# jojolebarjos/board-game-simulator-python

Hardware: AMD Instinct MI355X
Metric: env-steps/sec, Connect4(6,7,4) random rollout, batch=2^20 per GPU (higher is better)
Workload: dtype u64

## Files before the change

board-game-simulator-python_amd/csrc/bgs_host.hip:

```cpp
#include <immintrin.h>
#include <limits.h>
#include <linux/futex.h>
#include <pthread.h>
#include <sched.h>
#include <sys/syscall.h>
#include <time.h>
#include <unistd.h>

#include <atomic>
#include <chrono>
#include <condition_variable>
#include <cstdlib>
#include <cstdio>
#include <algorithm>
#include <cstring>
#include <mutex>
#include <new>
#include <thread>
#include <vector>

#include "bgs_capi_util.h"
#include "bgs_common.h"
#include "bgs_internal.h"

struct bgs_event {
    int device;
    hipEvent_t ev;
};

namespace {

using bgs::fail;

struct ExpandTable {
    uint64_t pairs[256];
    ExpandTable() {
        for (int byte = 0; byte < 256; ++byte) {
            uint64_t four = 0;
            for (int j = 0; j < 4; ++j) four |= (uint64_t)bgs::reward_pair((uint32_t)(byte >> (2 * j)) & 3u) << (16 * j);
            pairs[byte] = four;
        }
    }
};
const ExpandTable g_expand;

template <bool STREAM>
__attribute__((target("avx2"))) int64_t expand_avx2(const uint8_t* src, int64_t code_bytes, int8_t* dst) {
    const __m256i spread = _mm256_setr_epi8(0, 0, 0, 0, 1, 1, 1, 1, 2, 2, 2, 2, 3, 3, 3, 3,
                                            4, 4, 4, 4, 5, 5, 5, 5, 6, 6, 6, 6, 7, 7, 7, 7);
    const __m256i field = _mm256_set1_epi32((int)0xC0300C03u);
    const __m256i one = _mm256_set1_epi32(0x40100401);
    const __m256i two = _mm256_set1_epi32((int)0x80200802u);
    int64_t i = 0;
    for (; i + 8 <= code_bytes; i += 8) {
        long long eight;
        memcpy(&eight, src + i, 8);
        const __m256i rep = _mm256_shuffle_epi8(_mm256_set1_epi64x(eight), spread);
        const __m256i f = _mm256_and_si256(rep, field);
        const __m256i is1 = _mm256_cmpeq_epi8(f, one), is2 = _mm256_cmpeq_epi8(f, two);
        const __m256i r0 = _mm256_sub_epi8(is2, is1), r1 = _mm256_sub_epi8(is1, is2);
        const __m256i lo = _mm256_unpacklo_epi8(r0, r1), hi = _mm256_unpackhi_epi8(r0, r1);
        const __m256i first = _mm256_permute2x128_si256(lo, hi, 0x20), second = _mm256_permute2x128_si256(lo, hi, 0x31);
        if (STREAM) {
            _mm256_stream_si256(reinterpret_cast<__m256i*>(dst + 8 * i), first);
            _mm256_stream_si256(reinterpret_cast<__m256i*>(dst + 8 * i + 32), second);
        } else {
            _mm256_storeu_si256(reinterpret_cast<__m256i*>(dst + 8 * i), first);
            _mm256_storeu_si256(reinterpret_cast<__m256i*>(dst + 8 * i + 32), second);
        }
    }
    if (STREAM) _mm_sfence();
    return i;
}

const bool g_have_avx2 = __builtin_cpu_supports("avx2");
const bool g_stream_stores = bgs::experiment("no_stream_stores") == nullptr;
// ... 122 lines not shown
    while (seen < value && !a->compare_exchange_weak(seen, value, std::memory_order_release, std::memory_order_relaxed)) {
    }
    if (seen < value) futex(word, FUTEX_WAKE, INT_MAX, nullptr);
}

bool device_node_cpus(int device, cpu_set_t* out) {
    CPU_ZERO(out);
    char bus[64] = {0};
    if (hipDeviceGetPCIBusId(bus, (int)sizeof bus, device) != hipSuccess) return false;
    for (char* c = bus; *c; ++c) *c = (char)tolower(*c);
    char path[256];
    snprintf(path, sizeof path, "/sys/bus/pci/devices/%s/numa_node", bus);
    FILE* f = fopen(path, "r");
    if (!f) return false;
    int node = -1;
    const int got = fscanf(f, "%d", &node);
    fclose(f);
    if (got != 1 || node < 0) return false;
    snprintf(path, sizeof path, "/sys/devices/system/node/node%d/cpulist", node);
    f = fopen(path, "r");
    if (!f) return false;
    char list[4096] = {0};
    const bool have = fgets(list, sizeof list, f) != nullptr;
    fclose(f);
    if (!have) return false;
    cpu_set_t allowed;
    if (sched_getaffinity(0, sizeof allowed, &allowed) != 0) return false;
    int any = 0;
    char* save = nullptr;
    for (char* tok = strtok_r(list, ",\n", &save); tok; tok = strtok_r(nullptr, ",\n", &save)) {
        int lo = 0, hi = 0;
        const int k = sscanf(tok, "%d-%d", &lo, &hi);
        if (k < 1) continue;
        if (k == 1) hi = lo;
        for (int c = lo; c <= hi && c < CPU_SETSIZE; ++c)
            if (CPU_ISSET(c, &allowed)) {
                CPU_SET(c, out);
                ++any;
            }
    }
    return any > 0;
}

}

namespace {
inline bool sink_trace_on() {
    static const bool on = bgs::experiment("sink_trace") != nullptr;
    return on;
}
inline double mono_us() {
    return std::chrono::duration<double, std::micro>(std::chrono::steady_clock::now().time_since_epoch()).count();
}
}

static bool codes_hold_a_zero(const uint8_t* codes, int64_t first, int64_t count) {
    const uint8_t* p = codes + first / 4;
    const int64_t whole = count / 4;
    int64_t i = 0;
    uint64_t seen = 0;
    for (; i + 8 <= whole; i += 8) {
        uint64_t x;
        memcpy(&x, p + i, 8);
        seen |= ~(x | (x >> 1)) & 0x5555555555555555ull;
    }
    for (; i < whole; ++i) seen |= (uint64_t)(~(p[i] | (p[i] >> 1)) & 0x55u);
    for (int64_t k = 0; k < count - whole * 4; ++k) seen |= ((p[whole] >> (2 * k)) & 3u) == 0u ? 1u : 0u;
    return seen != 0;
}

struct bgs_reward_sink {
    int device = 0;
    int64_t max_games = 0;
    int slots = 0;
    int ring = 0;
    int threads = 0;
    std::vector<uint8_t*> pinned;
    std::vector<uint8_t*> mapped;
    std::vector<hipEvent_t> landed;
    bool grids = false;
    CellFormat cells;
    size_t slot_bytes = 0;
    struct Job {
        int64_t n_games = 0;
        int8_t* host_reward = nullptr;
        int event_slot = 0;
        bool all_end = false;
    };
    std::vector<Job> jobs;
    std::mutex mu;
    std::condition_variable cv_submit;
    std::condition_variable cv_landed;
    std::condition_variable cv_done;
    int64_t claimed = 0;
    int64_t submitted = 0;
    volatile int64_t* progress = nullptr;
    int64_t landed_upto = 0;
    int64_t completed = 0;
    std::vector<int> parts_done;
    std::vector<char> slot_ok;
    bool stop = false;
    std::vector<int64_t> failed_tickets;
    bool poll = false;
    std::vector<std::thread> workers;
    std::atomic<int64_t> a_submitted{0}, a_landed{0}, a_completed{0};
    std::atomic<bool> a_stop{false};
    std::atomic<int> urgent{0};
    int spin_us = 0;
    int wait_spin_us = 200;

    bool spin_for(const std::atomic<int64_t>& counter, int64_t ticket) const {
        if (counter.load(std::memory_order_acquire) > ticket) return true;
        if (spin_us <= 0) return false;
        const auto until = std::chrono::steady_clock::now() + std::chrono::microseconds(spin_us);
        for (;;) {
            for (int i = 0; i < 64; ++i) {
                if (counter.load(std::memory_order_acquire) > ticket || a_stop.load(std::memory_order_relaxed)) return true;
                _mm_pause();
            }
            if (std::chrono::steady_clock::now() >= until) return false;
        }
// ... 7 lines not shown
            bool ok = true;
            if (t == 0) {
                spin_for(a_submitted, ticket);
                {
                    std::unique_lock<std::mutex> lock(mu);
                    cv_submit.wait(lock, [&] { return stop || submitted > ticket; });
                    if (submitted <= ticket) return;
                    job = jobs[slot];
                }
                if (job.n_games == 0) {
                    ok = false;
                } else if (poll || urgent.load(std::memory_order_relaxed) > 0) {
                    hipError_t e;
                    while ((e = hipEventQuery(landed[job.event_slot])) == hipErrorNotReady) _mm_pause();
                    ok = e == hipSuccess;
                } else {
                    ok = hipEventSynchronize(landed[job.event_slot]) == hipSuccess;
                }
                if (sink_trace_on()) fprintf(stderr, "sink-trace ticket %lld landed %.1f\n", (long long)ticket, mono_us());
                {
                    std::lock_guard<std::mutex> lock(mu);
                    if (!ok && job.n_games != 0) failed_tickets.push_back(ticket);
                    slot_ok[slot] = ok;
                    landed_upto = ticket + 1;
                    a_landed.store(ticket + 1, std::memory_order_release);
                }
                cv_landed.notify_all();
            } else {
                if (urgent.load(std::memory_order_relaxed) > 0) {
                    const auto until = std::chrono::steady_clock::now() + std::chrono::microseconds(2000);
                    while (a_landed.load(std::memory_order_acquire) <= ticket && !a_stop.load(std::memory_order_relaxed) &&
                           urgent.load(std::memory_order_relaxed) > 0 && std::chrono::steady_clock::now() < until)
                        for (int i = 0; i < 16; ++i) _mm_pause();
                } else {
                    spin_for(a_landed, ticket);
                }
                std::unique_lock<std::mutex> lock(mu);
                cv_landed.wait(lock, [&] { return stop || landed_upto > ticket; });
                if (landed_upto <= ticket) return;
                job = jobs[slot];
                ok = slot_ok[slot];
            }
            const int expanders = threads > 1 ? threads - 1 : 1;
            const int share = threads > 1 ? t - 1 : 0;
            if (threads > 1 && t == 0) continue;
            const double trace_t0 = sink_trace_on() ? mono_us() : 0.0;
            if (ok && grids) {
                const int64_t blocks = (job.n_games + 63) / 64;
                const int64_t g0 = blocks * share / expanders * 64;
                const int64_t g1 = share + 1 == expanders ? job.n_games : blocks * (share + 1) / expanders * 64;
                static const bool skip = bgs::experiment("grid_no_expand") != nullptr;
                if (g1 > g0 && !skip) expand_cells(pinned[slot], job.n_games, cells, g0, g1 - g0, job.host_reward);
            } else if (ok) {
                const int64_t bytes = (job.n_games + 3) / 4;
                const int64_t b0 = bytes * share / expanders, b1 = bytes * (share + 1) / expanders;
                const int64_t first = b0 * 4;
                int64_t count = b1 * 4 - first;
                if (first + count > job.n_games) count = job.n_games - first;
                if (count > 0) expand_range(pinned[slot], first, count, job.host_reward);
                if (count > 0 && job.all_end && codes_hold_a_zero(pinned[slot], first, count)) {
                    std::lock_guard<std::mutex> lock(mu);
                    if (std::find(failed_tickets.begin(), failed_tickets.end(), ticket) == failed_tickets.end()) failed_tickets.push_back(ticket);
                }
            }
            if (sink_trace_on()) fprintf(stderr, "sink-trace ticket %lld worker %d expand %.1f .. %.1f\n", (long long)ticket, t, trace_t0, mono_us());
            {
                std::lock_guard<std::mutex> lock(mu);
                if (++parts_done[slot] == expanders) {
                    parts_done[slot] = 0;
                    ++completed;
                    a_completed.store(completed, std::memory_order_release);
                    cv_done.notify_all();
                    if (progress) progress_store_max(progress, completed);
                }
            }
        }
    }
};

namespace {

int64_t claim(bgs_reward_sink* s, bool ahead = false) {
    const int bound = ahead ? s->ring : s->slots;
    s->spin_for(s->a_completed, s->a_submitted.load(std::memory_order_relaxed) - bound);
    std::unique_lock<std::mutex> lock(s->mu);
    s->cv_done.wait(lock, [&] { return s->claimed - s->completed < bound; });
    return s->claimed++;
}

void publish(bgs_reward_sink* s, int64_t ticket, int64_t n_games, int8_t* host_reward, bool ok = true, int64_t event_ticket = -1,
             bool all_end = false) {
    {
        std::unique_lock<std::mutex> lock(s->mu);
        s->cv_done.wait(lock, [&] { return s->submitted == ticket; });
        s->jobs[ticket % s->ring].n_games = ok ? n_games : 0;
        s->jobs[ticket % s->ring].all_end = all_end;
        s->jobs[ticket % s->ring].host_reward = host_reward;
        s->jobs[ticket % s->ring].event_slot = (int)((event_ticket >= 0 ? event_ticket : ticket) % s->ring);
        if (!ok) s->failed_tickets.push_back(ticket);
        s->submitted = ticket + 1;
        s->a_submitted.store(ticket + 1, std::memory_order_release);
    }
    s->cv_submit.notify_one();
    s->cv_done.notify_all();
}

}

namespace bgs {
int64_t sink_claim(bgs_reward_sink* s) { return claim(s); }
uint8_t* sink_slot_device(bgs_reward_sink* s, int64_t ticket) { return s->mapped[ticket % s->ring]; }
uint8_t* sink_slot_host(bgs_reward_sink* s, int64_t ticket) { return s->pinned[ticket % s->ring]; }
hipEvent_t sink_slot_event(bgs_reward_sink* s, int64_t ticket) { return s->landed[ticket % s->ring]; }
void sink_publish(bgs_reward_sink* s, int64_t ticket, int64_t n_games, int8_t* host_reward, bool ok, int64_t event_ticket, bool all_end) {
    publish(s, ticket, n_games, host_reward, ok, event_ticket, all_end);
}
bool sink_takes_group(const bgs_reward_sink* s, int count) { return s != nullptr && !s->grids && count <= s->ring; }
int sink_ring(const bgs_reward_sink* s) { return s->ring; }
int sink_rollout_group(bgs_reward_sink* s, bgs_batch* const* bs, const uint64_t* seeds, const bool* writes, int count,
                       hipStream_t stream, int8_t* const* host_rewards, int64_t* tickets) {
    NEED(count >= 1 && count <= kConnectGroupMax && count <= s->ring && !s->grids, "bad step group");
    for (int i = 0; i < count; ++i)
        NEED(bs[i]->device == s->device && bs[i]->n <= s->max_games, "the batch does not fit the sink");
    uint32_t* codes[kConnectGroupMax];
    for (int i = 0; i < count; ++i) {
        tickets[i] = claim(s, true);
        codes[i] = reinterpret_cast<uint32_t*>(s->mapped[tickets[i] % s->ring]);
    }
    connect_rollout_steps(bs, seeds, codes, writes, count, stream);
    hipError_t err = hipGetLastError();
    if (err == hipSuccess) err = hipEventRecord(s->landed[tickets[count - 1] % s->ring], stream);
    for (int i = 0; i < count; ++i) publish(s, tickets[i], bs[i]->n, host_rewards[i], err == hipSuccess, tickets[count - 1]);
    if (err != hipSuccess) return fail(BGS_ERR_RUNTIME, "grouped rollout could not be enqueued: %s", hipGetErrorString(err));
    return BGS_OK;
}
int sink_wait(bgs_reward_sink* s, int64_t ticket, bool urgent) {
    NEED(s != nullptr, "sink is NULL");
    NEED(ticket >= 0 && ticket < s->a_submitted.load(std::memory_order_acquire), "unknown ticket %lld", (long long)ticket);
    if (s->a_completed.load(std::memory_order_acquire) <= ticket) {
        if (urgent) {
            s->urgent.fetch_add(1, std::memory_order_relaxed);
            const auto until = std::chrono::steady_clock::now() + std::chrono::microseconds(s->wait_spin_us);
            while (s->a_completed.load(std::memory_order_acquire) <= ticket && std::chrono::steady_clock::now() < until)
                for (int i = 0; i < 32; ++i) _mm_pause();
        } else {
            s->spin_for(s->a_completed, ticket);
        }
        {
            std::unique_lock<std::mutex> lock(s->mu);
            s->cv_done.wait(lock, [&] { return s->completed > ticket; });
        }
        if (urgent) s->urgent.fetch_sub(1, std::memory_order_relaxed);
    }
    int64_t bad = -1;
    {
        std::lock_guard<std::mutex> lock(s->mu);
        auto& f = s->failed_tickets;
        for (size_t i = 0; i < f.size();) {
            if (f[i] <= ticket) {
                if (bad < 0 || f[i] < bad) bad = f[i];
                f.erase(f.begin() + (long)i);
            } else {
                ++i;
            }
        }
    }
    if (bad >= 0)
        return fail(BGS_ERR_RUNTIME, "reward hand-over %lld failed (its enqueue, its arrival event, or -- a gathered step whose games all "
                    "had to end -- a rank delivered games that are still running: its step failed there); later deliveries are unaffected",
                    (long long)bad);
    return BGS_OK;
}
}

extern "C" {

int bgs_host_alloc(size_t bytes, void** host_ptr) {
    NEED(host_ptr != nullptr && bytes > 0, "bad argument");
    *host_ptr = nullptr;
    HIP_TRY(hipHostMalloc(host_ptr, bytes, hipHostMallocDefault));
    return BGS_OK;
}

int bgs_host_free(void* host_ptr) {
// ... 407 lines not shown
```

board-game-simulator-python_amd/csrc/bgs_internal.h:

```cpp
#pragma once

#include <hip/hip_runtime.h>
#include <stdint.h>
#include <stddef.h>

struct bgs_reward_sink;
struct bgs_gather;

enum { BGS_GAME_CONNECT = 1, BGS_GAME_BOUNCE = 2 };

#include "connect_unit.h"
#include "bounce_unit.h"

struct bgs_batch {
    int game;
    int generic;
    int gen_h, gen_w, gen_k;
    uint32_t gen_init_status;
    int device;
    int64_t n;
    hipStream_t stream;
    uint64_t first_game;
    ConnectGeom cg;
    BounceGeom bg;
    int planes;
    int num_cus;
    int rollout_wps;
    int bounce_group;
    int bounce_group_auto;
    int bounce_pieces;
    int bounce_flat_wps;
    int bounce_eval_wps;
    int bounce_flat_waves;
    int bounce_pool;
    int bounce_pieces_park;
    int bounce_park;
    int bounce_flat_chunk;
    int launches_in_flight;
    int bounce_memo_cold, bounce_memo_bypass;
    int bounce_epoch_limit;
    int bounce_wave_pass;
    int bounce_plan_auto;
    int bounce_passes;
    uint32_t bounce_pass_cap[BGS_BOUNCE_MAX_PASSES];
    int bounce_pass_group[BGS_BOUNCE_MAX_PASSES];
    int bounce_wave_grid;
    int transition_wave;
    int bounce_static_geom;
    int rollout_generic;
    int rollout_chunk;
    int rollout_opening;
    int rollout_no_lds;
    int rng_per_ply;
    void* arena;
    size_t arena_bytes;
    bool owns_arena;
    uint64_t* d_planes;
    uint8_t* d_status;
    uint16_t* d_plies;
    int8_t* d_reward;
    unsigned long long* d_steps;
    uint8_t* d_staging;
    size_t staging_bytes;
    uint64_t* d_gen_masks;
    int8_t* d_gen_cfg;
    uint32_t* d_worklist;
    uint32_t* d_work_count;
    uint32_t* d_pool;
    const uint32_t* book_links;
    const void* book_table;
    int book_depth;
    uint32_t book_n0;
    void* book_owner;
    void* pinned[2];
    hipEvent_t pinned_done[2];
    hipEvent_t order_event;
};

namespace bgs {

#ifdef BGS_TEST_HOOKS
const char* experiment(const char* name);
#else
inline const char* experiment(const char*) { return nullptr; }
#endif

void connect_reset(const bgs_batch* b);
void connect_step_random(const bgs_batch* b, uint64_t seed, uint32_t count);
void connect_step_actions(const bgs_batch* b, const int32_t* d_actions, int32_t* d_status_out);
bool connect_step_observe(const bgs_batch* b, const int32_t* d_actions, int32_t* d_status_out, uint8_t* d_legal, uint8_t* d_ended,
                          int8_t* d_reward_out, bool auto_reset);
void connect_reset_ended(const bgs_batch* b);
void bounce_reset_ended(const bgs_batch* b);
void status_to_ended(const bgs_batch* b, uint8_t* d_ended);
void connect_transition(const bgs_batch* b, const int32_t* d_actions, int32_t* d_status_out, int8_t* d_grid, int8_t* d_player,
                        int8_t* d_winner, int32_t* d_plies, uint8_t* d_legal, int8_t* d_reward_out, uint32_t* d_done = nullptr,
                        uint32_t ticket = 0);
bool connect_rollout(const bgs_batch* b, uint64_t seed, int32_t max_plies, uint32_t flags, uint32_t* codes_out);
bool connect_steps_ok(const bgs_batch* b, int32_t max_plies, uint32_t flags, bool codes);
void connect_rollout_steps(const bgs_batch* const* bs, const uint64_t* seeds, uint32_t* const* codes, const bool* writes, int count,
                           hipStream_t stream);
void connect_unpack_grid(const bgs_batch* b, int8_t* d_grid);
void connect_cell_planes(const bgs_batch* b, uint64_t* d_dst);
void connect_meta(const bgs_batch* b, int8_t* d_player, uint8_t* d_ended, int8_t* d_winner, int32_t* d_plies);
void connect_legal(const bgs_batch* b, uint8_t* d_legal, int32_t* d_count);
void connect_pack(const bgs_batch* b, const int8_t* d_grid, const int8_t* d_player, const int8_t* d_winner,
                  int32_t* d_status_out);

void connect_evaluate(const bgs_batch* b, uint64_t seed, int32_t playouts, int32_t max_plies, int32_t* d_counts, int policy);
int32_t connect_halving_min_budget(int width);
void connect_evaluate_halving(const bgs_batch* b, uint64_t seed, int32_t budget, int32_t max_plies, int policy, int32_t* d_counts,
                              int32_t* d_given, int32_t* d_best);
uint64_t connect_search_root_bytes(int width, int32_t iterations);
void connect_search(const bgs_batch* b, uint64_t seed, int32_t iterations, int32_t leaf_playouts, int32_t explore, int32_t max_plies,
                    int policy, int32_t* d_counts, int32_t* d_visits, int32_t* d_best, int32_t* d_nodes, void* d_workspace);
void connect_search_proving(const bgs_batch* b, uint64_t seed, int32_t iterations, int32_t leaf_playouts, int32_t explore,
                            int32_t max_plies, int policy, int32_t* d_counts, int32_t* d_visits, int32_t* d_best, int32_t* d_nodes,
                            int8_t* d_proved, int32_t* d_done, void* d_workspace);
uint64_t connect_forest_tree_bytes(int width, int32_t capacity);
void connect_forest_search(const bgs_batch* b, uint64_t seed, int32_t iterations, int32_t leaf_playouts, int32_t explore,
                           int32_t max_plies, int policy, int32_t capacity, int restart, int32_t* d_counts, int32_t* d_visits,
                           int32_t* d_best, int32_t* d_nodes, int32_t* d_carried, void* d_forest);
void connect_forest_advance(const bgs_batch* b, const int32_t* d_columns, int32_t capacity, int32_t* d_kept, void* d_forest);
uint64_t connect_guided_tree_bytes(int height, int width, int32_t capacity);
void connect_guided_step(const bgs_batch* b, int32_t capacity, int32_t cpuct, uint32_t flags, const float* d_priors,
                         const float* d_values, int8_t* d_leaf_grid, int8_t* d_leaf_player, int32_t* d_leaf_kind, int32_t* d_visits,
                         int32_t* d_scores, int32_t* d_best, int32_t* d_nodes, void* d_trees);
void connect_solve(const bgs_batch* b, int32_t depth, int64_t max_nodes, int8_t* d_codes, int16_t* d_plies,
                   unsigned long long* d_nodes);
void bounce_evaluate(const bgs_batch* b, uint64_t seed, int32_t playouts, int32_t max_plies, int32_t* d_counts, uint64_t* d_ends,
                     uint64_t* d_totals, int policy);
void bounce_evaluate_halving(const bgs_batch* b, uint64_t seed, int32_t budget, int32_t max_plies, int policy, int32_t* d_counts,
                             int32_t* d_given, int32_t* d_best);
uint64_t bounce_search_root_bytes(int32_t iterations, int32_t edges);
void bounce_search(const bgs_batch* b, uint64_t seed, int32_t iterations, int32_t leaf_playouts, int32_t explore, int32_t max_plies,
                   int policy, int32_t edges, int32_t* d_counts, int32_t* d_visits, int32_t* d_best, int32_t* d_nodes, int32_t* d_used,
                   void* d_workspace);
void bounce_search_proving(const bgs_batch* b, uint64_t seed, int32_t iterations, int32_t leaf_playouts, int32_t explore,
                           int32_t max_plies, int policy, int32_t edges, int32_t* d_counts, int32_t* d_visits, int32_t* d_best,
                           int32_t* d_nodes, int32_t* d_used, int8_t* d_proved, int32_t* d_done, void* d_workspace);
uint64_t bounce_forest_tree_bytes(int32_t capacity, int32_t edges);
void bounce_forest_search(const bgs_batch* b, uint64_t seed, int32_t iterations, int32_t leaf_playouts, int32_t explore,
                          int32_t max_plies, int policy, int32_t capacity, int32_t edges, int restart, int32_t* d_counts,
                          int32_t* d_visits, int32_t* d_best, int32_t* d_nodes, int32_t* d_used, int32_t* d_carried, void* d_forest);
void bounce_forest_advance(const bgs_batch* b, const int32_t* d_slots, int32_t capacity, int32_t edges, int32_t* d_kept, void* d_forest);
uint64_t bounce_guided_tree_bytes(int32_t capacity, int32_t edges);
void bounce_guided_step(const bgs_batch* b, int32_t capacity, int32_t edges, int32_t cpuct, int32_t max_plies, uint32_t flags,
                        const float* d_priors, const float* d_values, int8_t* d_leaf_grid, int8_t* d_leaf_player, int32_t* d_leaf_kind,
                        uint64_t* d_leaf_targets, int32_t* d_visits, int32_t* d_scores, int32_t* d_best, int32_t* d_nodes, int32_t* d_used,
                        void* d_trees);
void bounce_solve(const bgs_batch* b, int32_t depth, int64_t max_nodes, int8_t* d_codes, int16_t* d_plies, unsigned long long* d_nodes,
                  uint64_t* d_ends, uint64_t* d_totals);

void bounce_reset(const bgs_batch* b);
// ... 45 lines not shown
```

board-game-simulator-python_amd/csrc/connect_kernels.hip:

```cpp
#include <type_traits>

#include "bgs_common.h"
#include "bgs_internal.h"
#include "connect_board.h"

#ifndef BGS_TU_ID
#define BGS_TU_ID "unknown"
#endif
extern "C" const char bgs_tu_id_connect[] = BGS_TU_ID;

namespace bgs {
namespace {

template <int NW_, int SH, int SW, int SK>
struct Geo {
    static constexpr int NW = NW_;
    static constexpr int STATIC_H = SH, STATIC_W = SW, STATIC_K = SK;
    static constexpr int MAXW = SW ? SW : BGS_CONNECT_MAX_W;
    int rh, rw, rk;
    __device__ __forceinline__ int h() const { return SH ? SH : rh; }
    __device__ __forceinline__ int w() const { return SW ? SW : rw; }
    __device__ __forceinline__ int k() const { return SK ? SK : rk; }
    __device__ __forceinline__ uint32_t all_columns() const { return (1u << w()) - 1u; }
};
// ... 996 lines not shown
    plies.cheap(g, 3u, opening_draw<PER_PLY, 3>(own, words[0]), q, h4);
    if (OPEN_BLOCKS >= 2) {
        if constexpr (PER_PLY) own = philox4x32_10(seed, id, 1u);
        plies.cheap(g, 0u, opening_draw<PER_PLY, 0>(own, words[1]), q, h4);
        plies.cheap(g, 1u, opening_draw<PER_PLY, 1>(own, words[1]), q, h4);
        op = (h4 >> 3) & plies.ONES;
        plies.template full<2>(g, opening_draw<PER_PLY, 2>(own, words[1]), q, h4, op, alive, won_any);
        plies.template full<3>(g, opening_draw<PER_PLY, 3>(own, words[1]), q, h4, op, alive, won_any);
    }
#pragma unroll
    for (int ob = 2; ob < OPEN_BLOCKS; ++ob) {
        if constexpr (PER_PLY) own = philox4x32_10(seed, id, (uint32_t)ob);
        plies.template full<0>(g, opening_draw<PER_PLY, 0>(own, words[ob]), q, h4, op, alive, won_any);
        plies.template full<1>(g, opening_draw<PER_PLY, 1>(own, words[ob]), q, h4, op, alive, won_any);
        plies.template full<2>(g, opening_draw<PER_PLY, 2>(own, words[ob]), q, h4, op, alive, won_any);
        plies.template full<3>(g, opening_draw<PER_PLY, 3>(own, words[ob]), q, h4, op, alive, won_any);
    }
    if (OPEN_BLOCKS >= 2 && og < avail && alive == 0) {
        if (BOARDS || plane0) {
            plane0[og] = q[0];
            plane1[og] = q[1];
        }
        outcome[og] = (uint8_t)plies.outcome_of(q, won_any);
    }
    const uint32_t slot = og & (Pool::SLOTS - 1u);
    pool.plane[0][slot] = q[0];
    pool.plane[1][slot] = q[1];
    pool.cols[slot] = alive ? h4 : 0u;
#pragma unroll
    for (int k = 0; k < OW::QUADS; ++k) {
        auto at = [&](int i) { return OPEN_BLOCKS + i <= 11 ? words[OPEN_BLOCKS + i <= 11 ? OPEN_BLOCKS + i : 11] : 0u; };
        pool.words[k][slot] = make_uint4(at(4 * k), at(4 * k + 1), at(4 * k + 2), at(4 * k + 3));
    }
}

template <int QUADS, class Pool>
__device__ __forceinline__ void take_slot(const Pool& pool, uint32_t slot, uint64_t (&p)[2], uint32_t& hts, uint32_t& wnext,
                                          uint32_t* my_words) {
    p[0] = pool.plane[0][slot];
    p[1] = pool.plane[1][slot];
    hts = pool.cols[slot];
#pragma unroll
    for (int k = 0; k < QUADS; ++k) {
        const uint4 v = pool.words[k][slot];
        if (k == 0) wnext = v.x; else my_words[(4 * k) * BGS_WAVE] = v.x;
        my_words[(4 * k + 1) * BGS_WAVE] = v.y;
        my_words[(4 * k + 2) * BGS_WAVE] = v.z;
        my_words[(4 * k + 3) * BGS_WAVE] = v.w;
    }
}

template <bool CODES, bool ROLLED>
__device__ __forceinline__ uint32_t flush_outcomes(const uint32_t* outcome, uint32_t lane, uint32_t avail, bool boards,
                                                   uint8_t* status_out, uint16_t* reward_out, uint8_t* packed_out) {
    uint32_t stepped = 0;
    auto four_games = [&](uint32_t g4) {
        const ConnectOutcome4 o = connect_outcome4(outcome[g4 >> 2]);
        stepped += o.plies;
        if (CODES) packed_out[g4 >> 2] = (uint8_t)o.codes;
        if (!boards) return;
        if (g4 + 4u <= avail) {
            *reinterpret_cast<uint32_t*>(status_out + g4) = o.status;
            *reinterpret_cast<uint2*>(reward_out + g4) = make_uint2(o.reward[0], o.reward[1]);
        } else {
            for (uint32_t k = 0; g4 + k < avail; ++k) {
                status_out[g4 + k] = (uint8_t)(o.status >> (8u * k));
                reward_out[g4 + k] = (uint16_t)((((uint64_t)o.reward[1] << 32) | o.reward[0]) >> (16u * k));
            }
        }
    };
    if constexpr (ROLLED) {
#pragma unroll 1
        for (uint32_t g4 = lane * 4u; g4 < avail; g4 += BGS_WAVE * 4u) four_games(g4);
    } else {
        for (uint32_t g4 = lane * 4u; g4 < avail; g4 += BGS_WAVE * 4u) four_games(g4);
    }
    return stepped;
}

template <class G, int OPEN_BLOCKS, bool CODES, bool PER_PLY>
__global__ void __launch_bounds__(BGS_BLOCK)
k_connect_rollout_opened(G g, uint64_t* __restrict__ planes, uint8_t* __restrict__ status, uint16_t* __restrict__ reward,
                         int64_t n, uint64_t seed, uint64_t first_game, unsigned long long* __restrict__ steps,
                         uint32_t games_per_wave, uint32_t* __restrict__ codes_out) {
    using OW = OpenedWords<G, OPEN_BLOCKS, PER_PLY>;
    constexpr int NWORDS = OW::QUADS * 4;
    using Pool = OpenedPool<OW::QUADS>;
    constexpr bool DEFER = deferred_opening<G, OPEN_BLOCKS, PER_PLY>();
    static_assert(!DEFER || NWORDS == 8, "a replayed game refills rows 5 .. 7 with the words of blocks 8 .. 10");
    extern __shared__ uint32_t code_lds[];
    __shared__ Pool pools[BGS_BLOCK / BGS_WAVE];
    __shared__ uint32_t lane_words[BGS_BLOCK / BGS_WAVE][NWORDS][BGS_WAVE];
    const NibblePlies<G> plies(g);

    const uint32_t wave = __builtin_amdgcn_readfirstlane(blockIdx.x * (BGS_BLOCK / BGS_WAVE) + (threadIdx.x >> 6));
    const uint32_t lane = threadIdx.x & 63u;
    const int64_t begin = (int64_t)wave * games_per_wave;
    const int64_t end = begin + games_per_wave < n ? begin + games_per_wave : n;
    const uint32_t avail = begin < end ? (uint32_t)(end - begin) : 0u;
    uint32_t taken = 0;
    uint32_t opened = 0;
    uint64_t* __restrict__ const plane0 = planes + begin;
    uint64_t* __restrict__ const plane1 = planes + n + begin;
    Pool& pool = pools[threadIdx.x >> 6];

    uint64_t p[2] = {0, 0};
    uint32_t hts = 0, live = 0, game = 0;
    bool anywon = false;
    uint32_t wnext = 0;
    uint32_t* const my_words = &lane_words[threadIdx.x >> 6][0][lane];
    uint32_t wrow = 0;
    uint32_t myblk = 0;

    if (avail == 0u) return;
    uint8_t* const outcome = reinterpret_cast<uint8_t*>(code_lds + (threadIdx.x >> 6) * (games_per_wave >> 2));
    for (uint32_t i = lane; i < ((avail + 3u) >> 2); i += BGS_WAVE) reinterpret_cast<uint32_t*>(outcome)[i] = 0u;
    __builtin_amdgcn_wave_barrier();

    auto refetch = [&](uint64_t lane_seed, uint64_t id) {
        if (wrow == (kReplayRow | 7u)) {
            if (live != 0u) {
                const Philox4 d = philox4x32_10(lane_seed, id, 2u);
                my_words[5 * BGS_WAVE] = d.v[0];
                my_words[6 * BGS_WAVE] = d.v[1];
// ... 25 lines not shown
        plies.template full<1>(g, opening_draw<PER_PLY, 1>(four, word), p, hts, open, live, anywon);
        plies.template full<2>(g, opening_draw<PER_PLY, 2>(four, word), p, hts, open, live, anywon);
        plies.template full<3>(g, opening_draw<PER_PLY, 3>(four, word), p, hts, open, live, anywon);
        if (was_live != 0 && live == 0) {
            *reinterpret_cast<uint64_t*>(reinterpret_cast<char*>(plane0) + (game * 8u)) = p[0];
            *reinterpret_cast<uint64_t*>(reinterpret_cast<char*>(plane1) + (game * 8u)) = p[1];
            outcome[game] = (uint8_t)plies.outcome_of(p, anywon);
        }
    };
    auto take = [&](uint32_t which) {
        game = which;
        take_slot<PER_PLY ? 0 : OW::QUADS>(pool, which & (Pool::SLOTS - 1u), p, hts, wnext, my_words);
        if constexpr (PER_PLY) myblk = (uint32_t)OPEN_BLOCKS;
        wrow = DEFER ? 1u | ((hts << 3) & kReplayRow) : 1u;
        anywon = false;
        live = hts != 0u ? ~0u : 0u;
    };
    auto open_games = [&]() {
        const uint32_t og = opened + lane;
        const uint64_t id = first_game + (uint64_t)(begin + og);
        if constexpr (DEFER) open_games_deferred(g, pool, og & (Pool::SLOTS - 1u), seed, id, og < avail);
        else open_games_per_ply<OPEN_BLOCKS, PER_PLY, true>(g, plies, pool, seed, id, og, avail, plane0, plane1, outcome);
        opened += 64u;
    };

    while (taken < avail) {
        const uint64_t need = __builtin_amdgcn_ballot_w64(live == 0);
        if (need) {
            const uint32_t wanted = (uint32_t)__popcll(need);
            const uint32_t rank = __builtin_amdgcn_mbcnt_hi((uint32_t)(need >> 32), __builtin_amdgcn_mbcnt_lo((uint32_t)need, 0u));
            const uint32_t have = opened - taken;
            if (wanted > have && opened < avail) {
                const bool first = live == 0 && rank < have;
                const bool second = live == 0 && !first;
                if (first && taken + rank < avail) take(taken + rank);
                __builtin_amdgcn_fence(__ATOMIC_ACQ_REL, "wavefront");
                __builtin_amdgcn_wave_barrier();
                open_games();
                __builtin_amdgcn_fence(__ATOMIC_ACQ_REL, "wavefront");
                __builtin_amdgcn_wave_barrier();
                if (second && taken + rank < avail) take(taken + rank);
            } else if (live == 0 && taken + rank < avail) {
                take(taken + rank);
            }
            taken = avail - taken < wanted ? avail : taken + wanted;
        }
        play_block();
    }
    while (__builtin_amdgcn_ballot_w64(live != 0)) play_block();

    __builtin_amdgcn_fence(__ATOMIC_ACQ_REL, "wavefront");
    __builtin_amdgcn_wave_barrier();
    add_steps(steps, flush_outcomes<CODES, false>(reinterpret_cast<const uint32_t*>(outcome), lane, avail, true, status + begin,
                                                  reward + begin, reinterpret_cast<uint8_t*>(codes_out) + (begin >> 2)));
}

template <class G, int OPEN_BLOCKS, bool CODES>
__global__ void __launch_bounds__(BGS_BLOCK)
k_connect_rollout_opened_steps(G g, const ConnectGroup tab, int64_t n, uint32_t games_per_wave) {
    using OW = OpenedWords<G, OPEN_BLOCKS, false>;
    constexpr int NWORDS = OW::QUADS * 4;
    using Pool = OpenedPool<OW::QUADS>;
    constexpr bool DEFER = deferred_opening<G, OPEN_BLOCKS, false>();
    static_assert(!DEFER || NWORDS == 8, "a replayed game refills rows 5 .. 7 with the words of blocks 8 .. 10");
    extern __shared__ uint32_t code_lds[];
    __shared__ Pool pools[BGS_BLOCK / BGS_WAVE];
    __shared__ uint32_t lane_words[BGS_BLOCK / BGS_WAVE][NWORDS][BGS_WAVE];
    const NibblePlies<G> plies(g);

    const uint32_t wave = __builtin_amdgcn_readfirstlane(blockIdx.x * (BGS_BLOCK / BGS_WAVE) + (threadIdx.x >> 6));
    const uint32_t lane = threadIdx.x & 63u;
    const int64_t begin = (int64_t)wave * games_per_wave;
    const int64_t end = begin + games_per_wave < n ? begin + games_per_wave : n;
    const uint32_t avail = begin < end ? (uint32_t)(end - begin) : 0u;
    const uint32_t nsteps = (uint32_t)tab.count;
    uint32_t taken = 0, opened = 0;
    Pool& pool = pools[threadIdx.x >> 6];

    uint32_t cur = 0;
    bool pending = false;
    uint64_t cur_seed = tab.step[0].seed, cur_first = tab.step[0].first_game;
    uint64_t* cur_planes = tab.step[0].planes ? tab.step[0].planes + begin : nullptr;
    uint64_t* prev_planes = nullptr;
    uint64_t prev_seed = 0, prev_first = 0;

    uint64_t p[2] = {0, 0};
    uint32_t hts = 0, live = 0;
    uint32_t game = 0;
    uint32_t old = 0;
    bool anywon = false;
    uint32_t wnext = 0;
    uint32_t* const my_words = &lane_words[threadIdx.x >> 6][0][lane];
    uint32_t wrow = 0;

    if (avail == 0u) return;
    uint8_t* const outcome_bytes = reinterpret_cast<uint8_t*>(code_lds);
    const uint32_t slices_at = __builtin_amdgcn_readfirstlane((threadIdx.x >> 6) * 2u * games_per_wave);
    auto slice_at = [&](uint32_t s) { return slices_at + (s & 1u) * games_per_wave; };
    auto slice_of = [&](uint32_t s) { return outcome_bytes + slice_at(s); };
    uint32_t cur_at = slice_at(0u), prev_at = 0;
    auto zero_slice = [&](uint32_t s) {
        uint32_t* const w = reinterpret_cast<uint32_t*>(slice_of(s));
        for (uint32_t i = lane; i < ((avail + 3u) >> 2); i += BGS_WAVE) w[i] = 0u;
        __builtin_amdgcn_fence(__ATOMIC_ACQ_REL, "wavefront");
        __builtin_amdgcn_wave_barrier();
    };
    zero_slice(0u);

    auto refetch = [&]() {
        const bool at = wrow == (kReplayRow | 7u);
#pragma unroll
        for (uint32_t o = 0; o < 2u; ++o) {
            const bool here = at && live != 0u && old == o;
            if (__builtin_amdgcn_ballot_w64(here) == 0) continue;
            if (here) {
                const Philox4 d = philox4x32_10(o ? prev_seed : cur_seed,
                                                (o ? prev_first : cur_first) + (uint64_t)(begin + (game - (o ? prev_at : cur_at))), 2u);
                my_words[5 * BGS_WAVE] = d.v[0];
                my_words[6 * BGS_WAVE] = d.v[1];
                my_words[7 * BGS_WAVE] = d.v[2];
            }
        }
        if (at) wrow = 5u;
    };
    auto play_block = [&]() {
        const uint32_t was_live = live;
        const uint32_t word = wnext;
        if constexpr (DEFER) {
            if (__builtin_amdgcn_ballot_w64(wrow == (kReplayRow | 7u))) refetch();
            wnext = my_words[wrow * BGS_WAVE];
            const int32_t up = (int32_t)(wrow + 1u);
            wrow = (uint32_t)(up < NWORDS - 1 ? up : NWORDS - 1);
        } else {
            wnext = my_words[wrow * BGS_WAVE];
            wrow = wrow + 1u < (uint32_t)NWORDS - 1u ? wrow + 1u : (uint32_t)NWORDS - 1u;
        }
        uint32_t open = (hts >> 3) & plies.ONES;
        plies.template full<0>(g, sub_draw<0>(word), p, hts, open, live, anywon);
        plies.template full<1>(g, sub_draw<1>(word), p, hts, open, live, anywon);
        plies.template full<2>(g, sub_draw<2>(word), p, hts, open, live, anywon);
        plies.template full<3>(g, sub_draw<3>(word), p, hts, open, live, anywon);
        if (was_live != 0 && live == 0) {
            if (cur_planes != nullptr || prev_planes != nullptr) {
                uint64_t* const planes = old ? prev_planes : cur_planes;
                if (planes) {
                    const uint32_t at = (game - (old ? prev_at : cur_at)) * 8u;
                    *reinterpret_cast<uint64_t*>(reinterpret_cast<char*>(planes) + at) = p[0];
                    *reinterpret_cast<uint64_t*>(reinterpret_cast<char*>(planes + n) + at) = p[1];
                }
            }
            outcome_bytes[game] = (uint8_t)plies.outcome_of(p, anywon);
        }
    };
    auto take = [&](uint32_t which) {
        game = cur_at + which;
        old = 0u;
        take_slot<OW::QUADS>(pool, which & (Pool::SLOTS - 1u), p, hts, wnext, my_words);
        wrow = DEFER ? 1u | ((hts << 3) & kReplayRow) : 1u;
        anywon = false;
        live = hts != 0u ? ~0u : 0u;
    };
    auto open_games = [&]() {
        const uint32_t og = opened + lane;
        const uint64_t id = cur_first + (uint64_t)(begin + og);
        if constexpr (DEFER) open_games_deferred(g, pool, og & (Pool::SLOTS - 1u), cur_seed, id, og < avail);
        else open_games_per_ply<OPEN_BLOCKS, false, false>(g, plies, pool, cur_seed, id, og, avail, cur_planes,
                                                               cur_planes ? cur_planes + n : nullptr, slice_of(cur));
        opened += 64u;
    };
    auto flush = [&](uint32_t s) {
        __builtin_amdgcn_fence(__ATOMIC_ACQ_REL, "wavefront");
        __builtin_amdgcn_wave_barrier();
        const ConnectGroupStep& e = tab.step[s];
        const uint32_t stepped = flush_outcomes<CODES, true>(reinterpret_cast<const uint32_t*>(slice_of(s)), lane, avail,
                                                             e.planes != nullptr, e.status + begin, e.reward + begin,
                                                             reinterpret_cast<uint8_t*>(e.codes) + (begin >> 2));
        add_steps(e.steps, stepped);
    };
    auto flush_done = [&]() {
        if (pending && __builtin_amdgcn_ballot_w64(live != 0 && old != 0) == 0) {
            flush(cur - 1u);
            pending = false;
            prev_planes = nullptr;
        }
    };

    while (taken < avail || cur + 1u < nsteps) {
        const uint64_t need = __builtin_amdgcn_ballot_w64(live == 0);
        if (need) {
            const bool needy = live == 0;
            const uint32_t wanted = (uint32_t)__popcll(need);
            const uint32_t rank = __builtin_amdgcn_mbcnt_hi((uint32_t)(need >> 32), __builtin_amdgcn_mbcnt_lo((uint32_t)need, 0u));
            const uint32_t have = opened - taken;
            if (wanted > have && opened < avail) {
                const bool first = needy && rank < have;
                const bool second = needy && !first;
                if (first && taken + rank < avail) take(taken + rank);
                __builtin_amdgcn_fence(__ATOMIC_ACQ_REL, "wavefront");
                __builtin_amdgcn_wave_barrier();
                open_games();
                __builtin_amdgcn_fence(__ATOMIC_ACQ_REL, "wavefront");
                __builtin_amdgcn_wave_barrier();
                if (second && taken + rank < avail) take(taken + rank);
            } else if (needy && taken + rank < avail) {
                take(taken + rank);
            }
            const uint32_t served = avail - taken < wanted ? avail - taken : wanted;
            taken += served;
            if (served < wanted && cur + 1u < nsteps && !pending) {
                old = 1u;
                prev_planes = cur_planes;
                prev_seed = cur_seed;
                prev_first = cur_first;
                prev_at = cur_at;
                cur = __builtin_amdgcn_readfirstlane(cur + 1u);
                cur_at = slice_at(cur);
                pending = true;
                cur_seed = tab.step[cur].seed;
                cur_first = tab.step[cur].first_game;
                cur_planes = tab.step[cur].planes ? tab.step[cur].planes + begin : nullptr;
                zero_slice(cur);
                taken = 0;
                opened = 0;
                open_games();
                __builtin_amdgcn_fence(__ATOMIC_ACQ_REL, "wavefront");
                __builtin_amdgcn_wave_barrier();
                if (needy && rank >= served && rank - served < avail) take(rank - served);
                taken = avail < wanted - served ? avail : wanted - served;
            }
        }
        play_block();
        flush_done();
    }
    while (__builtin_amdgcn_ballot_w64(live != 0)) {
        play_block();
        flush_done();
    }
    if (pending) flush(cur - 1u);
    flush(cur);
}

template <class G, bool CAPPED>
__global__ void __launch_bounds__(BGS_BLOCK)
k_connect_rollout_aligned_wide(G g, uint64_t* __restrict__ planes, uint8_t* __restrict__ status,
                               uint16_t* __restrict__ reward, int64_t n, uint64_t seed, uint64_t first_game,
                               uint32_t max_plies, unsigned long long* __restrict__ steps, uint32_t games_per_wave,
                               uint32_t per_ply) {
    constexpr int NW = G::NW;
    constexpr uint32_t ONES = 0x11111111u;
    const int h = g.h(), w = g.w();
    const uint32_t open_lo0 = w >= 8 ? ONES : (ONES & ((1u << (4 * w)) - 1u));
    const uint32_t open_hi0 = w <= 8 ? 0u : (w >= 16 ? ONES : (ONES & ((1u << (4 * (w - 8))) - 1u)));

    const uint32_t wave = __builtin_amdgcn_readfirstlane(blockIdx.x * (BGS_BLOCK / BGS_WAVE) + (threadIdx.x >> 6));
    const int64_t begin = (int64_t)wave * games_per_wave;
    const int64_t end = begin + games_per_wave < n ? begin + games_per_wave : n;
    const uint32_t avail = begin < end ? (uint32_t)(end - begin) : 0u;
    uint32_t taken = 0;

    Bits<NW> p[2] = {zero_bits<NW>(), zero_bits<NW>()};
    uint64_t hts = 0;
    uint32_t open_lo = 0, open_hi = 0;
    uint32_t blk = 0, st = 0, game = 0, stepped = 0;
    uint64_t live = 0;

    if (avail == 0u) return;
    do {
        const uint64_t need = __builtin_amdgcn_ballot_w64(live == 0);
        if (need && taken < avail) {
            const uint32_t rank = __builtin_amdgcn_mbcnt_hi((uint32_t)(need >> 32), __builtin_amdgcn_mbcnt_lo((uint32_t)need, 0u));
            if (live == 0 && taken + rank < avail) {
                game = taken + rank;
                p[0] = zero_bits<NW>();
                p[1] = zero_bits<NW>();
                hts = 0;
                open_lo = open_lo0;
                open_hi = open_hi0;
                blk = 0;
                st = 0;
                live = (!CAPPED || max_plies > 0u) ? 1u : 0u;
                if (CAPPED && live == 0) {
                    store_planes<NW>(planes, n, begin + game, p[0], p[1]);
                    status[begin + game] = 0;
                    reward[begin + game] = 0;
                }
            }
            const uint32_t wanted = (uint32_t)__popcll(need);
            taken = avail - taken < wanted ? avail : taken + wanted;
        }

        const uint64_t was_live = live;
        const Philox4 four = philox4x32_10(seed, first_game + (uint64_t)(begin + game), per_ply ? blk : blk >> 2);
// ... 697 lines not shown
        }
        if constexpr (LdsBoard<G>::fits && G::NW > 1) {
            if (!b->rollout_generic && !b->rollout_no_lds) {
                auto launch_lds = [&](auto capped_tag, auto entry_tag) {
                    with_tags([&](auto codes_tag, auto rng_tag) {
                        constexpr bool CODES = decltype(codes_tag)::value;
                        launch(k_connect_rollout_lds<G, decltype(capped_tag)::value, CODES, decltype(entry_tag)::value,
                                                     decltype(rng_tag)::value>,
                               LdsBoard<G>::lds_bytes + (CODES ? shape.code_lds : 0), cap, b->d_steps, per_wave,
                               CODES ? codes_out : nullptr, reinterpret_cast<const OpenedBoard*>(b->d_staging));
                    }, fuse_codes, per_ply);
                };
                constexpr bool can_open = G::STATIC_K > 0 && 2 * G::STATIC_K - 2 >= (int)kOpenedPlies &&
                                          G::STATIC_H >= (int)kOpenedPlies && G::STATIC_H <= 15;
                if (initial && !capped && can_open && G::NW <= 3 && b->rollout_opening &&
                    b->staging_bytes >= (size_t)b->n * sizeof(OpenedBoard)) {
                    with_tags([&](auto rng_tag) {
                        hipLaunchKernelGGL((k_connect_open_lds<G, decltype(rng_tag)::value>), dim3(grid_for(b->n)), dim3(BGS_BLOCK), 0,
                                           b->stream, g, reinterpret_cast<OpenedBoard*>(b->d_staging), b->n, seed, b->first_game,
                                           b->d_steps);
                    }, per_ply);
                    launch_lds(std::false_type{}, std::integral_constant<int, kEntryOpened>{});
                } else {
                    with_tags([&](auto capped_tag, auto initial_tag) {
                        launch_lds(capped_tag, std::integral_constant<int, decltype(initial_tag)::value ? kEntryInitial : kEntryMemory>{});
                    }, capped, initial);
                }
                fused = fuse_codes;
                return;
            }
        }
        if (initial && !b->rollout_generic) {
            with_tags([&](auto capped_tag) {
                launch(k_connect_rollout_aligned_wide<G, decltype(capped_tag)::value>, 0, cap, b->d_steps, per_wave,
                       per_ply ? 1u : 0u);
            }, capped);
            return;
        }
        launch_game(Tag<GenericGame<G>>{});
    });
    return fused;
}

bool connect_steps_ok(const bgs_batch* b, int32_t max_plies, uint32_t flags, bool codes) {
    if (b->game != BGS_GAME_CONNECT || b->generic || !(b->cg.h == 6 && b->cg.w == 7 && b->cg.k == 4)) return false;
    if ((flags & 4u) || b->rng_per_ply || b->rollout_generic || b->rollout_opening != kRolloutOpeningBlocks) return false;
    const ConnectLaunchShape shape = connect_launch_shape(b->n, b->num_cus, b->rollout_wps, b->rollout_chunk);
    const bool capped = max_plies < 0 || (uint32_t)max_plies < (uint32_t)(b->cg.h * b->cg.w);
    return connect_opened_ok(b->cg, flags & 1u, capped, b->rollout_opening, shape) && shape.outcome_lds2 <= kRolloutLdsLimit &&
           (!codes || shape.code_lds <= kRolloutLdsLimit);
}

void connect_rollout_steps(const bgs_batch* const* bs, const uint64_t* seeds, uint32_t* const* codes, const bool* writes, int count,
                           hipStream_t stream) {
    const bgs_batch* b = bs[0];
    const ConnectLaunchShape shape = connect_launch_shape(b->n, b->num_cus, b->rollout_wps, b->rollout_chunk);
    ConnectGroup tab = {};
    tab.count = count;
    for (int i = 0; i < count; ++i) {
        ConnectGroupStep& e = tab.step[i];
        e.seed = seeds[i];
        e.first_game = bs[i]->first_game;
        e.planes = writes[i] ? bs[i]->d_planes : nullptr;
        e.status = writes[i] ? bs[i]->d_status : nullptr;
        e.reward = writes[i] ? reinterpret_cast<uint16_t*>(bs[i]->d_reward) : nullptr;
        e.codes = codes ? codes[i] : nullptr;
        e.steps = bs[i]->d_steps;
    }
    using G = Geo<1, 6, 7, 4>;
    with_tags([&](auto codes_tag) {
        hipLaunchKernelGGL((k_connect_rollout_opened_steps<G, kRolloutOpeningBlocks, decltype(codes_tag)::value>), dim3(shape.blocks),
                           dim3(BGS_BLOCK), shape.outcome_lds2, stream, G{6, 7, 4}, tab, b->n, (uint32_t)shape.per_wave);
    }, codes != nullptr);
}

void connect_unpack_grid(const bgs_batch* b, int8_t* d_grid) {
    const size_t lds = (size_t)BGS_BLOCK * b->cg.h * b->cg.w;
    dispatch(b->cg, [&](auto g) {
        using G = decltype(g);
        hipLaunchKernelGGL((k_connect_unpack<G>), dim3(grid_for(b->n)), dim3(BGS_BLOCK), lds, b->stream, g, b->d_planes,
                           b->n, d_grid);
    });
}

void connect_cell_planes(const bgs_batch* b, uint64_t* d_dst) {
    const int nwc = (b->cg.h * b->cg.w + 63) / 64;
    dispatch(b->cg, [&](auto g) {
        using G = decltype(g);
        hipLaunchKernelGGL((k_connect_cell_planes<G>), dim3(grid_for(b->n)), dim3(BGS_BLOCK), 0, b->stream, g, b->d_planes, b->n,
                           d_dst, nwc);
    });
}

void connect_meta(const bgs_batch* b, int8_t* d_player, uint8_t* d_ended, int8_t* d_winner, int32_t* d_plies) {
    hipLaunchKernelGGL(k_connect_meta, dim3(grid_for(b->n)), dim3(BGS_BLOCK), 0, b->stream, b->cg, b->d_planes, b->d_status,
                       b->n, d_player, d_ended, d_winner, d_plies);
}

void connect_legal(const bgs_batch* b, uint8_t* d_legal, int32_t* d_count) {
    dispatch(b->cg, [&](auto g) {
        using G = decltype(g);
        hipLaunchKernelGGL((k_connect_legal<G>), dim3(grid_for(b->n)), dim3(BGS_BLOCK), 0, b->stream, g, b->d_planes,
                           b->d_status, b->n, d_legal, d_count);
    });
}

void connect_transition(const bgs_batch* b, const int32_t* d_actions, int32_t* d_status_out, int8_t* d_grid, int8_t* d_player,
                        int8_t* d_winner, int32_t* d_plies, uint8_t* d_legal, int8_t* d_reward_out, uint32_t* d_done,
                        uint32_t ticket) {
    dispatch(b->cg, [&](auto g) {
        using G = decltype(g);
        hipLaunchKernelGGL((k_connect_transition<G>), dim3(grid_for(b->n)), dim3(BGS_BLOCK), 0, b->stream, g, b->d_planes,
                           b->d_status, reinterpret_cast<uint16_t*>(b->d_reward), b->n, d_actions, d_status_out, b->d_steps,
                           d_grid, d_player, d_winner, d_plies, d_legal, reinterpret_cast<uint16_t*>(d_reward_out),
                           grid_for(b->n) == 1 ? d_done : nullptr, ticket);
    });
}

void connect_pack(const bgs_batch* b, const int8_t* d_grid, const int8_t* d_player, const int8_t* d_winner,
                  int32_t* d_status_out) {
    dispatch(b->cg, [&](auto g) {
        using G = decltype(g);
        hipLaunchKernelGGL((k_connect_pack<G>), dim3(grid_for(b->n)), dim3(BGS_BLOCK), 0, b->stream, g, b->d_planes,
                           b->d_status, reinterpret_cast<uint16_t*>(b->d_reward), b->n, d_grid, d_player, d_winner,
                           d_status_out);
// ... 5 lines not shown
```

Measured before the change: 1074 billion.

## Pack outcome codes into dwords via DPP and record completion event at launch

The code flush now combines four lanes' code bytes with DPP row shuffles, so one lane per quad stores a 32-bit word with system scope to the host-mapped buffer instead of each lane storing a byte. This cuts the number of small PCIe writes. The grouped rollout launch now uses hipExtLaunchKernelGGL with a stop event instead of a separate hipEventRecord, unless an experiment flag selects the old path. Code offsets are now computed per wave from games_per_wave/16, which assumes that value is a multiple of 16, and the share arithmetic moves to a new header.

Measured after the change: 1068 billion. About the same (-0.6%).

```diff
diff --git a/board-game-simulator-python_amd/csrc/bgs_host.hip b/board-game-simulator-python_amd/csrc/bgs_host.hip
--- a/board-game-simulator-python_amd/csrc/bgs_host.hip
+++ b/board-game-simulator-python_amd/csrc/bgs_host.hip
@@ -22,6 +22,7 @@
 #include "bgs_capi_util.h"
 #include "bgs_common.h"
 #include "bgs_internal.h"
+#include "sink_codes.h"
 
 struct bgs_event {
     int device;
@@ -250,21 +251,6 @@
 inline double mono_us() {
     return std::chrono::duration<double, std::micro>(std::chrono::steady_clock::now().time_since_epoch()).count();
 }
-}
-
-static bool codes_hold_a_zero(const uint8_t* codes, int64_t first, int64_t count) {
-    const uint8_t* p = codes + first / 4;
-    const int64_t whole = count / 4;
-    int64_t i = 0;
-    uint64_t seen = 0;
-    for (; i + 8 <= whole; i += 8) {
-        uint64_t x;
-        memcpy(&x, p + i, 8);
-        seen |= ~(x | (x >> 1)) & 0x5555555555555555ull;
-    }
-    for (; i < whole; ++i) seen |= (uint64_t)(~(p[i] | (p[i] >> 1)) & 0x55u);
-    for (int64_t k = 0; k < count - whole * 4; ++k) seen |= ((p[whole] >> (2 * k)) & 3u) == 0u ? 1u : 0u;
-    return seen != 0;
 }
 
 struct bgs_reward_sink {
@@ -378,13 +364,10 @@
                 static const bool skip = bgs::experiment("grid_no_expand") != nullptr;
                 if (g1 > g0 && !skip) expand_cells(pinned[slot], job.n_games, cells, g0, g1 - g0, job.host_reward);
             } else if (ok) {
-                const int64_t bytes = (job.n_games + 3) / 4;
-                const int64_t b0 = bytes * share / expanders, b1 = bytes * (share + 1) / expanders;
-                const int64_t first = b0 * 4;
-                int64_t count = b1 * 4 - first;
-                if (first + count > job.n_games) count = job.n_games - first;
+                const SinkGames g = sink_share_games(job.n_games, share, expanders);
+                const int64_t first = g.first, count = g.count;
                 if (count > 0) expand_range(pinned[slot], first, count, job.host_reward);
-                if (count > 0 && job.all_end && codes_hold_a_zero(pinned[slot], first, count)) {
+                if (count > 0 && job.all_end && sink_codes_hold_a_zero(pinned[slot], first, count)) {
                     std::lock_guard<std::mutex> lock(mu);
                     if (std::find(failed_tickets.begin(), failed_tickets.end(), ticket) == failed_tickets.end()) failed_tickets.push_back(ticket);
                 }
@@ -453,9 +436,11 @@
         tickets[i] = claim(s, true);
         codes[i] = reinterpret_cast<uint32_t*>(s->mapped[tickets[i] % s->ring]);
     }
-    connect_rollout_steps(bs, seeds, codes, writes, count, stream);
+    static const bool record = bgs::experiment("sink_ext_event") != nullptr && atoi(bgs::experiment("sink_ext_event")) == 0;
+    const hipEvent_t done = s->landed[tickets[count - 1] % s->ring];
+    connect_rollout_steps(bs, seeds, codes, writes, count, stream, record ? nullptr : done);
     hipError_t err = hipGetLastError();
-    if (err == hipSuccess) err = hipEventRecord(s->landed[tickets[count - 1] % s->ring], stream);
+    if (err == hipSuccess && record) err = hipEventRecord(done, stream);
     for (int i = 0; i < count; ++i) publish(s, tickets[i], bs[i]->n, host_rewards[i], err == hipSuccess, tickets[count - 1]);
     if (err != hipSuccess) return fail(BGS_ERR_RUNTIME, "grouped rollout could not be enqueued: %s", hipGetErrorString(err));
     return BGS_OK;
diff --git a/board-game-simulator-python_amd/csrc/bgs_internal.h b/board-game-simulator-python_amd/csrc/bgs_internal.h
--- a/board-game-simulator-python_amd/csrc/bgs_internal.h
+++ b/board-game-simulator-python_amd/csrc/bgs_internal.h
@@ -1,6 +1,7 @@
 #pragma once
 
 #include <hip/hip_runtime.h>
+#include <hip/hip_ext.h>
 #include <stdint.h>
 #include <stddef.h>
 
@@ -99,7 +100,7 @@
 bool connect_rollout(const bgs_batch* b, uint64_t seed, int32_t max_plies, uint32_t flags, uint32_t* codes_out);
 bool connect_steps_ok(const bgs_batch* b, int32_t max_plies, uint32_t flags, bool codes);
 void connect_rollout_steps(const bgs_batch* const* bs, const uint64_t* seeds, uint32_t* const* codes, const bool* writes, int count,
-                           hipStream_t stream);
+                           hipStream_t stream, hipEvent_t done = nullptr);
 void connect_unpack_grid(const bgs_batch* b, int8_t* d_grid);
 void connect_cell_planes(const bgs_batch* b, uint64_t* d_dst);
 void connect_meta(const bgs_batch* b, int8_t* d_player, uint8_t* d_ended, int8_t* d_winner, int32_t* d_plies);
diff --git a/board-game-simulator-python_amd/csrc/connect_kernels.hip b/board-game-simulator-python_amd/csrc/connect_kernels.hip
--- a/board-game-simulator-python_amd/csrc/connect_kernels.hip
+++ b/board-game-simulator-python_amd/csrc/connect_kernels.hip
@@ -1072,13 +1072,22 @@
 
 template <bool CODES, bool ROLLED>
 __device__ __forceinline__ uint32_t flush_outcomes(const uint32_t* outcome, uint32_t lane, uint32_t avail, bool boards,
-                                                   uint8_t* status_out, uint16_t* reward_out, uint8_t* packed_out) {
+                                                   uint8_t* status_out, uint16_t* reward_out, uint32_t* packed_out) {
     uint32_t stepped = 0;
     auto four_games = [&](uint32_t g4) {
-        const ConnectOutcome4 o = connect_outcome4(outcome[g4 >> 2]);
+        const bool in = !CODES || g4 < avail;
+        const ConnectOutcome4 o = connect_outcome4(in ? outcome[g4 >> 2] : 0u);
         stepped += o.plies;
-        if (CODES) packed_out[g4 >> 2] = (uint8_t)o.codes;
-        if (!boards) return;
+        if constexpr (CODES) {
+            constexpr int kQuad1133 = 1 | (1 << 2) | (3 << 4) | (3 << 6), kQuad2222 = 2 | (2 << 2) | (2 << 4) | (2 << 6);
+            uint32_t c = o.codes;
+            c |= (uint32_t)__builtin_amdgcn_update_dpp(0, (int)(c << 8), kQuad1133, 0xF, 0xF, true);
+            c |= (uint32_t)__builtin_amdgcn_update_dpp(0, (int)(c << 16), kQuad2222, 0xF, 0xF, true);
+            uint32_t me = lane;
+            asm volatile("" : "+v"(me));
+            if (in && (me & 3u) == 0u) __hip_atomic_store(packed_out + (g4 >> 4), c, __ATOMIC_RELAXED, __HIP_MEMORY_SCOPE_SYSTEM);
+        }
+        if (!boards || !in) return;
         if (g4 + 4u <= avail) {
             *reinterpret_cast<uint32_t*>(status_out + g4) = o.status;
             *reinterpret_cast<uint2*>(reward_out + g4) = make_uint2(o.reward[0], o.reward[1]);
@@ -1089,7 +1098,12 @@
             }
         }
     };
-    if constexpr (ROLLED) {
+    if constexpr (CODES && ROLLED) {
+#pragma unroll 1
+        for (uint32_t base = 0; base < avail; base += BGS_WAVE * 4u) four_games(base + lane * 4u);
+    } else if constexpr (CODES) {
+        for (uint32_t base = 0; base < avail; base += BGS_WAVE * 4u) four_games(base + lane * 4u);
+    } else if constexpr (ROLLED) {
 #pragma unroll 1
         for (uint32_t g4 = lane * 4u; g4 < avail; g4 += BGS_WAVE * 4u) four_games(g4);
     } else {
@@ -1221,7 +1235,7 @@
     __builtin_amdgcn_fence(__ATOMIC_ACQ_REL, "wavefront");
     __builtin_amdgcn_wave_barrier();
     add_steps(steps, flush_outcomes<CODES, false>(reinterpret_cast<const uint32_t*>(outcome), lane, avail, true, status + begin,
-                                                  reward + begin, reinterpret_cast<uint8_t*>(codes_out) + (begin >> 2)));
+                                                  reward + begin, codes_out + (begin >> 4)));
 }
 
 template <class G, int OPEN_BLOCKS, bool CODES>
@@ -1242,6 +1256,7 @@
     const int64_t begin = (int64_t)wave * games_per_wave;
     const int64_t end = begin + games_per_wave < n ? begin + games_per_wave : n;
     const uint32_t avail = begin < end ? (uint32_t)(end - begin) : 0u;
+    const uint32_t codes_at = wave * (games_per_wave >> 4);
     const uint32_t nsteps = (uint32_t)tab.count;
     uint32_t taken = 0, opened = 0;
     Pool& pool = pools[threadIdx.x >> 6];
@@ -1343,7 +1358,7 @@
         const ConnectGroupStep& e = tab.step[s];
         const uint32_t stepped = flush_outcomes<CODES, true>(reinterpret_cast<const uint32_t*>(slice_of(s)), lane, avail,
                                                              e.planes != nullptr, e.status + begin, e.reward + begin,
-                                                             reinterpret_cast<uint8_t*>(e.codes) + (begin >> 2));
+                                                             e.codes + codes_at);
         add_steps(e.steps, stepped);
     };
     auto flush_done = [&]() {
@@ -1405,8 +1420,7 @@
         play_block();
         flush_done();
     }
-    if (pending) flush(cur - 1u);
-    flush(cur);
+    for (uint32_t s = pending ? cur - 1u : cur; s <= cur; ++s) flush(s);
 }
 
 template <class G, bool CAPPED>
@@ -2210,7 +2224,7 @@
 }
 
 void connect_rollout_steps(const bgs_batch* const* bs, const uint64_t* seeds, uint32_t* const* codes, const bool* writes, int count,
-                           hipStream_t stream) {
+                           hipStream_t stream, hipEvent_t done) {
     const bgs_batch* b = bs[0];
     const ConnectLaunchShape shape = connect_launch_shape(b->n, b->num_cus, b->rollout_wps, b->rollout_chunk);
     ConnectGroup tab = {};
@@ -2227,8 +2241,9 @@
     }
     using G = Geo<1, 6, 7, 4>;
     with_tags([&](auto codes_tag) {
-        hipLaunchKernelGGL((k_connect_rollout_opened_steps<G, kRolloutOpeningBlocks, decltype(codes_tag)::value>), dim3(shape.blocks),
-                           dim3(BGS_BLOCK), shape.outcome_lds2, stream, G{6, 7, 4}, tab, b->n, (uint32_t)shape.per_wave);
+        hipExtLaunchKernelGGL((k_connect_rollout_opened_steps<G, kRolloutOpeningBlocks, decltype(codes_tag)::value>),
+                              dim3(shape.blocks), dim3(BGS_BLOCK), shape.outcome_lds2, stream, nullptr, done, 0, G{6, 7, 4}, tab,
+                              b->n, (uint32_t)shape.per_wave);
     }, codes != nullptr);
 }
 
diff --git a/board-game-simulator-python_amd/csrc/sink_codes.h b/board-game-simulator-python_amd/csrc/sink_codes.h
--- /dev/null
+++ b/board-game-simulator-python_amd/csrc/sink_codes.h
@@ -0,0 +1,37 @@
+#pragma once
+
+#include <stdint.h>
+#include <string.h>
+
+struct SinkBytes {
+    int64_t b0, b1;
+};
+
+constexpr int64_t sink_code_bytes(int64_t n_games) { return (n_games + 3) / 4; }
+constexpr SinkBytes sink_share(int64_t n_games, int share, int expanders) {
+    const int64_t bytes = sink_code_bytes(n_games);
+    return SinkBytes{bytes * share / expanders, bytes * (share + 1) / expanders};
+}
+struct SinkGames {
+    int64_t first, count;
+};
+constexpr SinkGames sink_share_games(int64_t n_games, int share, int expanders) {
+    const SinkBytes r = sink_share(n_games, share, expanders);
+    const int64_t first = r.b0 * 4;
+    const int64_t end = r.b1 * 4 < n_games ? r.b1 * 4 : n_games;
+    return SinkGames{first, end > first ? end - first : 0};
+}
+inline bool sink_codes_hold_a_zero(const uint8_t* codes, int64_t first, int64_t count) {
+    const uint8_t* p = codes + first / 4;
+    const int64_t whole = count / 4;
+    int64_t i = 0;
+    uint64_t seen = 0;
+    for (; i + 8 <= whole; i += 8) {
+        uint64_t x;
+        memcpy(&x, p + i, 8);
+        seen |= ~(x | (x >> 1)) & 0x5555555555555555ull;
+    }
+    for (; i < whole; ++i) seen |= (uint64_t)(~(p[i] | (p[i] >> 1)) & 0x55u);
+    for (int64_t k = 0; k < count - whole * 4; ++k) seen |= ((p[whole] >> (2 * k)) & 3u) == 0u ? 1u : 0u;
+    return seen != 0;
+}
```
